# kr4b/pigs

Measured on AMD Instinct MI355X. Metric: sample-points/sec (fwd + 1st + 2nd derivatives, fused), higher is better.
Workload: dtype f32; 1 GPU; c3: 65536 Gaussians x 1024x1024 grid, 1024 rows x 1024 points per GPU, d=2, c=1, kappa=0.5, orders 0-2; gaussians=65536, points_per_gpu=1048576, step=preprocess (cold: nothing reused) + fused forward (orders 0..2)

## Files before the change

pigs_amd/csrc/plan_forward.h:

```cpp
#pragma once
#include "plan_lists.h"

#ifndef PIGS_FWD_WAVES
#define PIGS_FWD_WAVES 8
#endif
#ifndef PIGS_FWD_WG_WAVES
#define PIGS_FWD_WG_WAVES 4
#endif
#ifndef PIGS_FWD_UNROLL
#define PIGS_FWD_UNROLL 2
#endif

namespace pigs {

struct Rec {
    float mu[2], con[3], v[2];
};

template <int STRIDE, typename Body>
__device__ __forceinline__ void walk_point(const PlanView& pv, float x, float y, int i, Body&& body) {
    const GaussGrid gg = pv.params->gg;
    const uint32_t level_mask = pv.params->level_mask;
    for (int l = 0; l < pv.L; ++l) {
        if (!(level_mask >> l & 1u)) continue;
        const int G = pv.G0 >> l;
        const float inv_s = gg.inv_s0 * __builtin_amdgcn_ldexpf(1.f, -l);
        const float gmax = (float)(G - 1);
        const int cx = (int)clampf(floorf((x - gg.ox) * inv_s), 0.f, gmax);
        const int cy = (int)clampf(floorf((y - gg.oy) * inv_s), 0.f, gmax);
        const int cx0 = cx > 0 ? cx - 1 : 0, cx1 = cx < G - 1 ? cx + 1 : G - 1;
        const int cy0 = cy > 0 ? cy - 1 : 0, cy1 = cy < G - 1 ? cy + 1 : G - 1;
        const int csh = level_shift((uint32_t)(G * G));
        uint32_t j0[3], j1[3];
#pragma unroll
        for (int r = 0; r < 3; ++r) {
            const int yy = cy0 + r;
            const uint32_t row = (uint32_t)((yy <= cy1 ? yy : cy1) * G);
            j0[r] = pv.starts[pv.level_off[l] + ((row + (uint32_t)cx0) << csh)];
            j1[r] = yy <= cy1 ? pv.starts[pv.level_off[l] + ((row + (uint32_t)cx1 + 1u) << csh)] : j0[r];
        }
#pragma unroll
        for (int r = 0; r < 3; ++r)
            for (uint32_t j = j0[r] + (uint32_t)i; j < j1[r]; j += STRIDE) body(j, pv.rec[2 * (size_t)j], pv.rec[2 * (size_t)j + 1]);
    }
}
template <typename Body>
__device__ __forceinline__ void walk_point_instep(const PlanView& pv, float x, float y, int i, Body&& body) {
    const GaussGrid gg = pv.params->gg;
    const uint32_t level_mask = pv.params->level_mask;
    for (int l = 0; l < pv.L; ++l) {
        if (!(level_mask >> l & 1u)) continue;
        const int G = pv.G0 >> l;
        const float inv_s = gg.inv_s0 * __builtin_amdgcn_ldexpf(1.f, -l);
        const float gmax = (float)(G - 1);
        const int cx = (int)clampf(floorf((x - gg.ox) * inv_s), 0.f, gmax);
        const int cy = (int)clampf(floorf((y - gg.oy) * inv_s), 0.f, gmax);
        const int cx0 = cx > 0 ? cx - 1 : 0, cx1 = cx < G - 1 ? cx + 1 : G - 1;
        const int cy0 = cy > 0 ? cy - 1 : 0, cy1 = cy < G - 1 ? cy + 1 : G - 1;
        const int csh = level_shift((uint32_t)(G * G));
        uint32_t j0[3], j1[3];
#pragma unroll
        for (int r = 0; r < 3; ++r) {
            const int yy = cy0 + r;
            const uint32_t row = (uint32_t)((yy <= cy1 ? yy : cy1) * G);
            j0[r] = pv.starts[pv.level_off[l] + ((row + (uint32_t)cx0) << csh)];
            j1[r] = yy <= cy1 ? pv.starts[pv.level_off[l] + ((row + (uint32_t)cx1 + 1u) << csh)] : j0[r];
        }
#pragma unroll
        for (int r = 0; r < 3; ++r) {
            uint32_t len = j1[r] - j0[r];
#pragma unroll
            for (int o = 16; o < 64; o <<= 1) len = max(len, (uint32_t)__shfl_xor((int)len, o));
            len = (uint32_t)__builtin_amdgcn_readfirstlane((int)len);
            for (uint32_t o = 0; o < len; o += 16u) {
                const uint32_t j = j0[r] + o + (uint32_t)i;
                const bool have = j < j1[r];
                const size_t jj = have ? j : pv.N;
                body(have, (uint32_t)jj, pv.rec[2 * jj], pv.rec[2 * jj + 1]);
            }
        }
    }
}
__device__ __forceinline__ float pair_q(const float4 A, const float4 B, float x, float y) {
    const float dx = x - A.x, dy = y - A.y;
    return A.z * dx * dx + (2.f * A.w * dx + B.x * dy) * dy;
}
__device__ __forceinline__ Rec make_rec(const float4 A, const float4 B) {
    Rec r;
    r.mu[0] = A.x; r.mu[1] = A.y; r.con[0] = A.z; r.con[1] = A.w; r.con[2] = B.x;
    r.v[0] = B.y; r.v[1] = B.z;
    return r;
}

template <int STEP, bool WIDE, typename Step, typename RangesMask>
__device__ __forceinline__ void for_each_step(const PlanView& pv, uint32_t tile, int lane, Step&& step,
                                              RangesMask&& ranges_mask) {
    const uint32_t hdr = pv.hdr[(size_t)tile * TILE_HDR_WORDS];
    const uint32_t count = hdr & TILE_COUNT_MASK;
    const uint32_t* slab = pv.tlist + (size_t)tile * pv.list_cap;
    if ((hdr >> TILE_MODE_SHIFT) == TILE_MODE_LIST) {
        for (uint32_t e0 = 0; e0 < count; e0 += STEP) {
            const bool have = lane < STEP && e0 + (uint32_t)lane < count;
            const uint32_t e = have ? slab[e0 + lane] : 0u;
            step(e & LIST_IDX_MASK, WIDE ? (e >> LIST_WIDE_SHIFT) & 15u : e >> LIST_NARROW_SHIFT, have);
        }
    } else if ((hdr >> TILE_MODE_SHIFT) == TILE_MODE_GROUPS) {
        for (uint32_t g = 0; g < 4; ++g) {
            const uint32_t ng = pv.hdr[(size_t)tile * TILE_HDR_WORDS + 1 + g];
            const uint32_t* gl = pv.glist + ((size_t)tile * 4 + g) * pv.list_cap;
            for (uint32_t e0 = 0; e0 < ng; e0 += STEP) {
                const bool have = lane < STEP && e0 + (uint32_t)lane < ng;
                step(have ? gl[e0 + lane] : 0u, have ? 1u << g : 0u, have);
            }
        }
    } else {
        auto mask = ranges_mask();
        for (uint32_t r = 0; r < count; ++r) {
            const uint32_t j0 = slab[2 * r], len = slab[2 * r + 1];
            for (uint32_t o = 0; o < len; o += STEP) {
                const bool have = lane < STEP && o + (uint32_t)lane < len;
                const uint32_t idx = have ? j0 + o + (uint32_t)lane : j0;
                step(idx, mask(idx, have), have);
            }
        }
    }
}

#ifndef PIGS_GROUP_CAP
#define PIGS_GROUP_CAP 32
#endif
constexpr int GROUP_CAP = PIGS_GROUP_CAP;
static_assert(GROUP_CAP >= 8 && GROUP_CAP % PIGS_FWD_UNROLL == 0, "queue capacity");

struct FwdLds {
    static constexpr int GSTRIDE = GROUP_CAP * 32 + 32;
    float4 rec[(4 * GSTRIDE + PIGS_FWD_UNROLL * 32) / 16];
};

typedef float f4v __attribute__((ext_vector_type(4)));
typedef float f2v __attribute__((ext_vector_type(2)));

__device__ __forceinline__ uint32_t lds_addr(const void* p) {
    return (uint32_t)(uintptr_t)(const __attribute__((address_space(3))) void*)p;
}
template <int C> struct LdsRec;
template <> struct LdsRec<1> { f4v a; f2v b; };
template <> struct LdsRec<2> { f4v a; f4v b; };
template <int OFF>
__device__ __forceinline__ void lds_rec_issue(LdsRec<1>& r, uint32_t addr) {
    asm volatile("ds_read_b128 %0, %2 offset:%3\n\tds_read_b64 %1, %2 offset:%4"
                 : "=v"(r.a), "=v"(r.b) : "v"(addr), "i"(OFF), "i"(OFF + 16));
}
template <int OFF>
__device__ __forceinline__ void lds_rec_issue(LdsRec<2>& r, uint32_t addr) {
    asm volatile("ds_read_b128 %0, %2 offset:%3\n\tds_read_b128 %1, %2 offset:%4"
                 : "=v"(r.a), "=v"(r.b) : "v"(addr), "i"(OFF), "i"(OFF + 16));
}
template <int C>
__device__ __forceinline__ void lds_rec_wait(LdsRec<C>* r) {
    asm volatile("s_waitcnt lgkmcnt(0)" : "+v"(r[0].a), "+v"(r[0].b), "+v"(r[1].a), "+v"(r[1].b));
}
template <int C>
__device__ __forceinline__ Rec rec_of(const LdsRec<C>& x) {
    Rec r;
    r.mu[0] = x.a.x; r.mu[1] = x.a.y; r.con[0] = x.a.z; r.con[1] = x.a.w; r.con[2] = x.b.x; r.v[0] = x.b.y;
    if constexpr (C == 2) r.v[1] = x.b.z;
    else r.v[1] = 0.f;
    return r;
}

template <int C, int MASK>
__device__ __forceinline__ void evaluate_rows(float* acc, const float* s, const FwdLds& lds, int rows, int lane,
                                              const RzOf<float, MASK>& rz) {
    static_assert(PIGS_FWD_UNROLL == 2, "two rows per register set");
    uint32_t q = lds_addr(lds.rec) + (uint32_t)(lane >> 4) * FwdLds::GSTRIDE;
    LdsRec<C> ra[2], rb[2];
    auto eval2 = [&](const LdsRec<C>* r) {
#pragma unroll
        for (int u = 0; u < 2; ++u) {
            const Rec x = rec_of<C>(r[u]);
            fwd_accumulate<float, 2, C, MASK>(acc, s, x.mu, x.con, x.v, &rz);
        }
    };
    lds_rec_issue<0>(ra[0], q);
    lds_rec_issue<32>(ra[1], q);
    int k = 0;
    for (; k + 4 <= rows; k += 4) {
        lds_rec_wait<C>(ra);
        lds_rec_issue<64>(rb[0], q);
        lds_rec_issue<96>(rb[1], q);
        eval2(ra);
        lds_rec_wait<C>(rb);
        lds_rec_issue<128>(ra[0], q);
        lds_rec_issue<160>(ra[1], q);
        q += 128;
        eval2(rb);
    }
    lds_rec_wait<C>(ra);
    if (k < rows) eval2(ra);
}

template <int C, int MASK>
constexpr int fwd_waves() {
    constexpr int n = FwdLayout<2, C, MASK>::N;
    if (MASK == ORDC) return 7;
    return n > 12 ? 4 : n > 10 ? 5 : (C == 1 && (MASK == 7 || MASK == 19 || MASK == 1 || MASK == ORDR || MASK == ORDG)) ? PIGS_FWD_WAVES : 6;
}
constexpr bool fwd_can_stage(int C, int MASK) { return C == 1 && (MASK == 7 || MASK == 19); }
template <int C, int MASK>
__device__ __forceinline__ void stage_store(const PlanView& pv, const float* acc, uint32_t m) {
    using L = FwdLayout<2, C, MASK>;
    if constexpr (C == 1 && MASK == 7) {
        pv.stage[2 * (size_t)m] = make_float4(acc[L::O0], -acc[L::O1], -acc[L::O1 + 1], acc[L::O2]);
        pv.stage[2 * (size_t)m + 1] = make_float4(acc[L::O2 + 1], acc[L::O2 + 1], acc[L::O2 + 2], 0.f);
    } else if constexpr (C == 1 && MASK == 19) {
        pv.stage[2 * (size_t)m] = make_float4(acc[L::O0], -acc[L::O1], -acc[L::O1 + 1], acc[L::O2]);
    }
}

template <int C, int MASK>
__device__ __forceinline__ void forward_points_quad(const PlanView& pv, const SamplesView& sv, uint32_t tile, uint32_t quad, int lane,
                                                    float q_f, float* __restrict__ o0, float* __restrict__ o1,
                                                    float* __restrict__ o2, float* __restrict__ o3, const RzOf<float, MASK>& rz) {
    using L = FwdLayout<2, C, MASK>;
    const int row = lane >> 4, i = lane & 15;
    const uint32_t m = tile * TILE_POINTS + quad * 4u + (uint32_t)row;
    const bool valid = m < sv.M;
    const SPoint sp = tile_point(sv, point_order(sv), tile, quad * 4u + (uint32_t)row);
    const float s[2] = {sp.x, sp.y};
    float acc[L::N];
#pragma unroll
    for (int k = 0; k < L::N; ++k) acc[k] = 0.f;
    walk_point<16>(pv, sp.x, sp.y, i, [&](uint32_t, const float4 A, const float4 B) {
        if (!(pair_q(A, B, sp.x, sp.y) > q_f)) {
            const Rec r = make_rec(A, B);
            fwd_accumulate<float, 2, C, MASK>(acc, s, r.mu, r.con, r.v, &rz);
        }
    });
#pragma unroll
    for (int k = 0; k < L::N; ++k) {
#pragma unroll
        for (int o = 1; o < 16; o <<= 1) acc[k] += __shfl_xor(acc[k], o);
    }
    if (i == 0 && valid) {
        if (fwd_can_stage(C, MASK) && pv.stage) stage_store<C, MASK>(pv, acc, sp.m);
        else fwd_store<float, 2, C, MASK, false>(acc, (int64_t)sp.m, o0, o1, o2, o3, &rz);
    }
}

template <int C, int MASK>
__device__ __forceinline__ void forward_tile(const PlanView& pv, const SamplesView& sv, uint32_t tile, int lane, FwdLds& lds,
                                             float* __restrict__ o0, float* __restrict__ o1, float* __restrict__ o2,
                                             float* __restrict__ o3, const RzOf<float, MASK>& rz) {
    using L = FwdLayout<2, C, MASK>;
    constexpr int U = PIGS_FWD_UNROLL;
    constexpr bool CAN_STAGE = fwd_can_stage(C, MASK);
    __builtin_amdgcn_s_setprio(3);
    char* const qbase = (char*)lds.rec;
    const uint32_t m = tile * TILE_POINTS + (uint32_t)lane;
    const bool valid = m < sv.M;
    const int g = lane >> 4, i = lane & 15;
    asm volatile("" ::"s"(sv.params), "s"(sv.M), "s"(pv.hdr), "s"(pv.glist), "s"(pv.list_cap));
    const PointOrderWords pw = point_order_words(sv);
    const uint32_t* hd = pv.hdr + (size_t)tile * TILE_HDR_WORDS;
    uint32_t zero = 0u;
    asm("" : "+v"(zero));
    const uint32_t h0v = hd[zero];
    const uint32_t ngv = hd[1 + g];
    const uint32_t* gl = pv.glist + ((size_t)tile * 4 + g) * pv.list_cap;
    uint32_t e0 = gl[(uint32_t)i < pv.list_cap ? i : 0], e1 = gl[16u + (uint32_t)i < pv.list_cap ? 16 + i : 0];
    const SPoint sp = tile_point(sv, point_order(pw), tile, (uint32_t)lane);
    const uint32_t h0 = (uint32_t)__builtin_amdgcn_readfirstlane((int)h0v);
    const float s[2] = {sp.x, sp.y};
    float acc[L::N];
#pragma unroll
    for (int k = 0; k < L::N; ++k) acc[k] = 0.f;
    auto chunk = [&](int rows, auto&& index_of) {
        static_assert(GROUP_CAP == 32, "two rounds of 16 records per chunk");
        rows = __builtin_amdgcn_readfirstlane((rows + U - 1) / U * U);
        const uint32_t j0 = index_of(0, i), j1 = index_of(1, 16 + i);
        const float4 A0 = pv.rec[2 * (size_t)j0], B0 = pv.rec[2 * (size_t)j0 + 1];
        float4 A1 = A0, B1 = B0;
        if (rows > 16) { A1 = pv.rec[2 * (size_t)j1]; B1 = pv.rec[2 * (size_t)j1 + 1]; }
        float4* dst = (float4*)(qbase + g * FwdLds::GSTRIDE + i * 32);
        wave_lds_fence();
        dst[0] = A0;
        *(float2*)(dst + 1) = make_float2(B0.x, B0.y);
        if constexpr (C == 2) *(float2*)((char*)(dst + 1) + 8) = make_float2(B0.z, 0.f);
        if (rows > 16) {
            dst[32] = A1;
            *(float2*)(dst + 33) = make_float2(B1.x, B1.y);
            if constexpr (C == 2) *(float2*)((char*)(dst + 33) + 8) = make_float2(B1.z, 0.f);
        }
        wave_lds_fence();
        __builtin_amdgcn_s_setprio(0);
        evaluate_rows<C, MASK>(acc, s, lds, rows, lane, rz);
        __builtin_amdgcn_s_setprio(3);
    };
    if ((h0 >> TILE_MODE_SHIFT) == TILE_MODE_POINTS) {
        return;
    } else if ((h0 >> TILE_MODE_SHIFT) != TILE_MODE_RANGES) {
        const uint32_t ng = ngv;
        const uint32_t n0 = (uint32_t)__builtin_amdgcn_readlane((int)ngv, 0), n1 = (uint32_t)__builtin_amdgcn_readlane((int)ngv, 16);
        const uint32_t n2 = (uint32_t)__builtin_amdgcn_readlane((int)ngv, 32), n3 = (uint32_t)__builtin_amdgcn_readlane((int)ngv, 48);
        uint32_t nmax = n0 > n1 ? n0 : n1;
        nmax = n2 > nmax ? n2 : nmax;
        nmax = n3 > nmax ? n3 : nmax;
        for (uint32_t base = 0; base < nmax; base += GROUP_CAP) {
            const int rows = (int)(nmax - base < GROUP_CAP ? nmax - base : GROUP_CAP);
            chunk(rows, [&](int round, int p) { return base + p < ng ? (round == 0 ? e0 : e1) : pv.N; });
            if (base + GROUP_CAP < nmax) {
                const uint32_t p0 = base + GROUP_CAP + (uint32_t)i, p1 = p0 + 16u;
                e0 = gl[p0 < pv.list_cap ? p0 : 0u];
                e1 = gl[p1 < pv.list_cap ? p1 : 0u];
            }
        }
    } else {
        const uint32_t* slab = pv.tlist + (size_t)tile * pv.list_cap;
        const uint32_t count = h0 & TILE_COUNT_MASK;
        const float INF = __builtin_huge_valf();
        const float q_f = pv.params->q_f;
        float x0 = valid ? sp.x : INF, x1 = valid ? sp.x : -INF, y0 = valid ? sp.y : INF, y1 = valid ? sp.y : -INF;
        row_box_dpp(x0, x1, y0, y1);
        const bool row_has_points = x0 <= x1;
        float4* const q = (float4*)(qbase + g * FwdLds::GSTRIDE);
        int qn = 0;
        auto drain = [&]() {
            int rows = qn;
#pragma unroll
            for (int o = 16; o < 64; o <<= 1) rows = max(rows, __shfl_xor(rows, o));
            rows = __builtin_amdgcn_readfirstlane((rows + U - 1) / U * U);
            wave_lds_fence();
            for (int k = qn + i; k < rows; k += 16) {
                q[2 * k] = make_float4(0.f, 0.f, 0.f, 0.f);
                q[2 * k + 1] = make_float4(0.f, 0.f, 0.f, 0.f);
            }
            wave_lds_fence();
            if (rows > 0) {
                __builtin_amdgcn_s_setprio(0);
                evaluate_rows<C, MASK>(acc, s, lds, rows, lane, rz);
                __builtin_amdgcn_s_setprio(3);
            }
            qn = 0;
        };
        for (uint32_t r = 0; r < count; ++r) {
            const uint32_t j0 = slab[2 * r], len = slab[2 * r + 1];
            for (uint32_t base = 0; base < len; base += 16) {
                const bool in = base + (uint32_t)i < len;
                const size_t j = in ? j0 + base + (uint32_t)i : pv.N;
                const float4 A = pv.rec[2 * j], B = pv.rec[2 * j + 1];
                const bool hit = in && row_has_points && ellipse_reaches_rect(ellipse_of(A, B.x), x0, y0, x1, y1, q_f);
                const uint32_t rm = (uint32_t)(__ballot(hit) >> (16 * g)) & 0xffffu;
                if (hit) {
                    const int k = qn + __builtin_popcount(rm & ((1u << i) - 1u));
                    q[2 * k] = A;
                    *(float2*)(q + 2 * k + 1) = make_float2(B.x, B.y);
                    if constexpr (C == 2) *(float2*)((char*)(q + 2 * k + 1) + 8) = make_float2(B.z, 0.f);
                }
                qn += __builtin_popcount(rm);
                if (__any(qn > GROUP_CAP - 16)) drain();
            }
        }
        drain();
    }
    const uint32_t m_other = (uint32_t)__shfl_xor((int)sp.m, 1);
    const uint32_t dist = sp.m > m_other ? sp.m - m_other : m_other - sp.m;
    const bool stream = __builtin_popcountll(__ballot(valid && dist == 1u)) >= 48;
    if (CAN_STAGE && pv.stage) {
        if (valid) stage_store<C, MASK>(pv, acc, sp.m);
    } else if (valid) {
        if (stream) {
            fwd_store<float, 2, C, MASK, true>(acc, (int64_t)sp.m, o0, o1, o2, o3, &rz);
            asm volatile("" ::: "memory");
        } else {
            fwd_store<float, 2, C, MASK, false>(acc, (int64_t)sp.m, o0, o1, o2, o3, &rz);
        }
    }
}

template <int C, int MASK>
__global__ __launch_bounds__(64 * PIGS_FWD_WG_WAVES, (fwd_waves<C, MASK>())) void tile_forward_kernel(
    PlanView pv, SamplesView sv, float* __restrict__ o0, float* __restrict__ o1, float* __restrict__ o2,
    float* __restrict__ o3, RzOf<float, MASK> rz) {
    constexpr uint32_t FW = PIGS_FWD_WG_WAVES;
    __shared__ FwdLds lds_all[FW];
    const int lane = threadIdx.x & 63;
    const int wave = __builtin_amdgcn_readfirstlane(threadIdx.x >> 6);
    const uint32_t nmain = (sv.ntiles + FW - 1u) / FW;
    constexpr uint32_t NHELP = POINT_HELPER_BLOCKS * 4u / FW;
    static_assert(NHELP % 8u == 0u, "the main workgroups keep their XCD");
    if (blockIdx.x < NHELP) {
        const uint32_t n = pv.params->n_points;
        if (n == 0u) return;
        const float q_f = pv.params->q_f;
        const uint32_t hw = blockIdx.x * FW + (uint32_t)wave, nhw = NHELP * FW;
        for (uint32_t qd = hw; qd < n * 16u; qd += nhw)
            forward_points_quad<C, MASK>(pv, sv, pv.ptiles[qd >> 4], qd & 15u, lane, q_f, o0, o1, o2, o3, rz);
        return;
    }
    const uint32_t tile = xcd_block_chunk<PIGS_XCD_CHUNK * 4 / FW>(nmain, blockIdx.x - NHELP) * FW + (uint32_t)wave;
    if (tile >= sv.ntiles) return;
    forward_tile<C, MASK>(pv, sv, tile, lane, lds_all[wave], o0, o1, o2, o3, rz);
}

template <int C, int MASK>
__global__ __launch_bounds__(256) void plan_lists_forward_kernel(ListArgs a, float* __restrict__ o0, float* __restrict__ o1,
                                                                 float* __restrict__ o2, float* __restrict__ o3, RzOf<float, MASK> rz) {
    __shared__ ListsLds<LISTS_TPW> lds_all[4];
    static_assert(sizeof(FwdLds) <= sizeof(ListsLds<LISTS_TPW>), "the forward's queues live in the list build's LDS");
    const int lane = threadIdx.x & 63;
    const int wave = __builtin_amdgcn_readfirstlane(threadIdx.x >> 6);
    lists_strip_cover(a);
    const uint32_t tile0 = lists_tile0<LISTS_TPW>(wave);
    const uint32_t ntiles = a.sv.ntiles;
    if (tile0 >= ntiles) return;
    build_block_lists<LISTS_TPW>(a, lds_all[wave], tile0, lane);
    __builtin_amdgcn_fence(__ATOMIC_RELEASE, "workgroup");
    __builtin_amdgcn_fence(__ATOMIC_ACQUIRE, "workgroup");
    FwdLds& flds = *reinterpret_cast<FwdLds*>(&lds_all[wave]);
    for (int t = 0; t < LISTS_TPW; ++t) {
        const uint32_t tile = tile0 + (uint32_t)t;
        if (tile >= ntiles) break;
        const uint32_t h0 = __hip_atomic_load(a.pv.hdr + (size_t)tile * TILE_HDR_WORDS, __ATOMIC_RELAXED, __HIP_MEMORY_SCOPE_WORKGROUP);
        if ((h0 >> TILE_MODE_SHIFT) == TILE_MODE_POINTS) {
            for (uint32_t quad = 0; quad < 16u; ++quad) forward_points_quad<C, MASK>(a.pv, a.sv, tile, quad, lane, a.q_f, o0, o1, o2, o3, rz);
        } else {
            forward_tile<C, MASK>(a.pv, a.sv, tile, lane, flds, o0, o1, o2, o3, rz);
        }
    }
}

template <int MASK>
__global__ __launch_bounds__(256) void stage_to_outputs_kernel(const float4* __restrict__ stage, uint32_t M, float* __restrict__ o0,
                                                               float* __restrict__ o1, float* __restrict__ o2) {
    const uint32_t m = blockIdx.x * 256 + threadIdx.x;
    if (m >= M) return;
    const float4 a = stage[2 * (size_t)m];
    if (o0) __builtin_nontemporal_store(a.x, &o0[m]);
    if (o1) { __builtin_nontemporal_store(a.y, &o1[2 * (size_t)m]); __builtin_nontemporal_store(a.z, &o1[2 * (size_t)m + 1]); }
    if constexpr (MASK == 7) {
        const float4 b = stage[2 * (size_t)m + 1];
        if (o2) {
            float* h = o2 + 4 * (size_t)m;
            __builtin_nontemporal_store(a.w, h); __builtin_nontemporal_store(b.x, h + 1);
            __builtin_nontemporal_store(b.y, h + 2); __builtin_nontemporal_store(b.z, h + 3);
        }
    } else {
        if (o2) __builtin_nontemporal_store(a.w, &o2[m]);
    }
}

}
```

Before: 22.70 billion sample-points/s.

## Stream Gaussian records into LDS via async global_load_lds with double-buffered rounds

Replaces the register-staged global-to-LDS copy of Gaussian records with direct global_load_lds DMA into an interleaved, split A/B layout. Rounds of 16 records are double-buffered, so the next round's load overlaps evaluation of the current one. The LDS layout changes to rows of four groups, and the list-index assignment moves from lane>>4 groups to lane&3 groups. It also adds an occupancy hint of 5 to the lists kernel. The split layout always copies the full 32-byte record including padding, and the vmcnt(0) waits may serialize other loads.

After: 22.86 billion sample-points/s, median of 6. About the same (+0.7%).

```diff
diff --git a/pigs_amd/csrc/plan_forward.h b/pigs_amd/csrc/plan_forward.h
--- a/pigs_amd/csrc/plan_forward.h
+++ b/pigs_amd/csrc/plan_forward.h
@@ -130,11 +130,14 @@
 #define PIGS_GROUP_CAP 32
 #endif
 constexpr int GROUP_CAP = PIGS_GROUP_CAP;
-static_assert(GROUP_CAP >= 8 && GROUP_CAP % PIGS_FWD_UNROLL == 0, "queue capacity");
+static_assert(GROUP_CAP == 32 && PIGS_FWD_UNROLL == 2, "two rounds of 16 records per queue, two rows per register set");
 
 struct FwdLds {
-    static constexpr int GSTRIDE = GROUP_CAP * 32 + 32;
-    float4 rec[(4 * GSTRIDE + PIGS_FWD_UNROLL * 32) / 16];
+    static constexpr int ROUND = 16;
+    static constexpr int ROW = 4 * 16;
+    static constexpr int SLAB = ROUND * ROW;
+    static constexpr int BOFF = GROUP_CAP / ROUND * SLAB;
+    float4 rec[(2 * BOFF + PIGS_FWD_UNROLL * ROW) / 16];
 };
 
 typedef float f4v __attribute__((ext_vector_type(4)));
@@ -149,12 +152,12 @@
 template <int OFF>
 __device__ __forceinline__ void lds_rec_issue(LdsRec<1>& r, uint32_t addr) {
     asm volatile("ds_read_b128 %0, %2 offset:%3\n\tds_read_b64 %1, %2 offset:%4"
-                 : "=v"(r.a), "=v"(r.b) : "v"(addr), "i"(OFF), "i"(OFF + 16));
+                 : "=v"(r.a), "=v"(r.b) : "v"(addr), "i"(OFF), "i"(OFF + FwdLds::BOFF));
 }
 template <int OFF>
 __device__ __forceinline__ void lds_rec_issue(LdsRec<2>& r, uint32_t addr) {
     asm volatile("ds_read_b128 %0, %2 offset:%3\n\tds_read_b128 %1, %2 offset:%4"
-                 : "=v"(r.a), "=v"(r.b) : "v"(addr), "i"(OFF), "i"(OFF + 16));
+                 : "=v"(r.a), "=v"(r.b) : "v"(addr), "i"(OFF), "i"(OFF + FwdLds::BOFF));
 }
 template <int C>
 __device__ __forceinline__ void lds_rec_wait(LdsRec<C>* r) {
@@ -169,11 +172,21 @@
     return r;
 }
 
-template <int C, int MASK>
-__device__ __forceinline__ void evaluate_rows(float* acc, const float* s, const FwdLds& lds, int rows, int lane,
+__device__ __forceinline__ void lds_round_dma(const float4* rec, FwdLds& lds, int round, uint32_t j) {
+    typedef const __attribute__((address_space(1))) void* gptr;
+    typedef __attribute__((address_space(3))) void* lptr;
+    const float4* src = rec + 2 * (size_t)j;
+    char* dst = (char*)lds.rec + round * FwdLds::SLAB;
+    __builtin_amdgcn_global_load_lds((gptr)src, (lptr)dst, 16, 0, 0);
+    __builtin_amdgcn_global_load_lds((gptr)src, (lptr)(dst + FwdLds::BOFF - 16), 16, 16, 0);
+}
+__device__ __forceinline__ void lds_dma_wait() { asm volatile("s_waitcnt vmcnt(0)" ::: "memory"); }
+
+template <int C, int MASK>
+__device__ __forceinline__ void evaluate_rows(float* acc, const float* s, const FwdLds& lds, int row0, int rows, int lane,
                                               const RzOf<float, MASK>& rz) {
-    static_assert(PIGS_FWD_UNROLL == 2, "two rows per register set");
-    uint32_t q = lds_addr(lds.rec) + (uint32_t)(lane >> 4) * FwdLds::GSTRIDE;
+    constexpr int R = FwdLds::ROW;
+    uint32_t q = lds_addr(lds.rec) + (uint32_t)row0 * R + (uint32_t)(lane >> 4) * 16u;
     LdsRec<C> ra[2], rb[2];
     auto eval2 = [&](const LdsRec<C>* r) {
 #pragma unroll
@@ -183,17 +196,17 @@
         }
     };
     lds_rec_issue<0>(ra[0], q);
-    lds_rec_issue<32>(ra[1], q);
+    lds_rec_issue<R>(ra[1], q);
     int k = 0;
     for (; k + 4 <= rows; k += 4) {
         lds_rec_wait<C>(ra);
-        lds_rec_issue<64>(rb[0], q);
-        lds_rec_issue<96>(rb[1], q);
+        lds_rec_issue<2 * R>(rb[0], q);
+        lds_rec_issue<3 * R>(rb[1], q);
         eval2(ra);
         lds_rec_wait<C>(rb);
-        lds_rec_issue<128>(ra[0], q);
-        lds_rec_issue<160>(ra[1], q);
-        q += 128;
+        lds_rec_issue<4 * R>(ra[0], q);
+        lds_rec_issue<5 * R>(ra[1], q);
+        q += 4 * R;
         eval2(rb);
     }
     lds_rec_wait<C>(ra);
@@ -260,60 +273,56 @@
     const uint32_t m = tile * TILE_POINTS + (uint32_t)lane;
     const bool valid = m < sv.M;
     const int g = lane >> 4, i = lane & 15;
+    const int kq = lane >> 2, gq = lane & 3;
     asm volatile("" ::"s"(sv.params), "s"(sv.M), "s"(pv.hdr), "s"(pv.glist), "s"(pv.list_cap));
     const PointOrderWords pw = point_order_words(sv);
     const uint32_t* hd = pv.hdr + (size_t)tile * TILE_HDR_WORDS;
     uint32_t zero = 0u;
     asm("" : "+v"(zero));
     const uint32_t h0v = hd[zero];
-    const uint32_t ngv = hd[1 + g];
-    const uint32_t* gl = pv.glist + ((size_t)tile * 4 + g) * pv.list_cap;
-    uint32_t e0 = gl[(uint32_t)i < pv.list_cap ? i : 0], e1 = gl[16u + (uint32_t)i < pv.list_cap ? 16 + i : 0];
+    const uint32_t ngv = hd[1 + gq];
+    const uint32_t* gl = pv.glist + ((size_t)tile * 4 + gq) * pv.list_cap;
+    uint32_t e0 = gl[(uint32_t)kq < pv.list_cap ? kq : 0], e1 = gl[16u + (uint32_t)kq < pv.list_cap ? 16 + kq : 0];
     const SPoint sp = tile_point(sv, point_order(pw), tile, (uint32_t)lane);
     const uint32_t h0 = (uint32_t)__builtin_amdgcn_readfirstlane((int)h0v);
     const float s[2] = {sp.x, sp.y};
     float acc[L::N];
 #pragma unroll
     for (int k = 0; k < L::N; ++k) acc[k] = 0.f;
-    auto chunk = [&](int rows, auto&& index_of) {
-        static_assert(GROUP_CAP == 32, "two rounds of 16 records per chunk");
-        rows = __builtin_amdgcn_readfirstlane((rows + U - 1) / U * U);
-        const uint32_t j0 = index_of(0, i), j1 = index_of(1, 16 + i);
-        const float4 A0 = pv.rec[2 * (size_t)j0], B0 = pv.rec[2 * (size_t)j0 + 1];
-        float4 A1 = A0, B1 = B0;
-        if (rows > 16) { A1 = pv.rec[2 * (size_t)j1]; B1 = pv.rec[2 * (size_t)j1 + 1]; }
-        float4* dst = (float4*)(qbase + g * FwdLds::GSTRIDE + i * 32);
-        wave_lds_fence();
-        dst[0] = A0;
-        *(float2*)(dst + 1) = make_float2(B0.x, B0.y);
-        if constexpr (C == 2) *(float2*)((char*)(dst + 1) + 8) = make_float2(B0.z, 0.f);
-        if (rows > 16) {
-            dst[32] = A1;
-            *(float2*)(dst + 33) = make_float2(B1.x, B1.y);
-            if constexpr (C == 2) *(float2*)((char*)(dst + 33) + 8) = make_float2(B1.z, 0.f);
-        }
-        wave_lds_fence();
+    auto evaluate = [&](int row0, int rows) {
         __builtin_amdgcn_s_setprio(0);
-        evaluate_rows<C, MASK>(acc, s, lds, rows, lane, rz);
+        evaluate_rows<C, MASK>(acc, s, lds, row0, rows, lane, rz);
         __builtin_amdgcn_s_setprio(3);
     };
     if ((h0 >> TILE_MODE_SHIFT) == TILE_MODE_POINTS) {
         return;
     } else if ((h0 >> TILE_MODE_SHIFT) != TILE_MODE_RANGES) {
         const uint32_t ng = ngv;
-        const uint32_t n0 = (uint32_t)__builtin_amdgcn_readlane((int)ngv, 0), n1 = (uint32_t)__builtin_amdgcn_readlane((int)ngv, 16);
-        const uint32_t n2 = (uint32_t)__builtin_amdgcn_readlane((int)ngv, 32), n3 = (uint32_t)__builtin_amdgcn_readlane((int)ngv, 48);
+        const uint32_t n0 = (uint32_t)__builtin_amdgcn_readlane((int)ngv, 0), n1 = (uint32_t)__builtin_amdgcn_readlane((int)ngv, 1);
+        const uint32_t n2 = (uint32_t)__builtin_amdgcn_readlane((int)ngv, 2), n3 = (uint32_t)__builtin_amdgcn_readlane((int)ngv, 3);
         uint32_t nmax = n0 > n1 ? n0 : n1;
         nmax = n2 > nmax ? n2 : nmax;
         nmax = n3 > nmax ? n3 : nmax;
-        for (uint32_t base = 0; base < nmax; base += GROUP_CAP) {
-            const int rows = (int)(nmax - base < GROUP_CAP ? nmax - base : GROUP_CAP);
-            chunk(rows, [&](int round, int p) { return base + p < ng ? (round == 0 ? e0 : e1) : pv.N; });
-            if (base + GROUP_CAP < nmax) {
-                const uint32_t p0 = base + GROUP_CAP + (uint32_t)i, p1 = p0 + 16u;
-                e0 = gl[p0 < pv.list_cap ? p0 : 0u];
-                e1 = gl[p1 < pv.list_cap ? p1 : 0u];
-            }
+        auto index_of = [&](uint32_t e, uint32_t p) { return p < ng ? e : pv.N; };
+        auto landed = [&]() {
+            lds_dma_wait();
+            asm volatile("" ::"v"(sp.x), "v"(sp.y), "v"(sp.m));
+        };
+        if (nmax > 0u) {
+            wave_lds_fence();
+            lds_round_dma(pv.rec, lds, 0, index_of(e0, (uint32_t)kq));
+            landed();
+        }
+        for (uint32_t base = 0; base < nmax; base += FwdLds::ROUND) {
+            const int rows = __builtin_amdgcn_readfirstlane((int)(nmax - base < FwdLds::ROUND ? (nmax - base + U - 1) / U * U : FwdLds::ROUND));
+            const uint32_t next = base + FwdLds::ROUND;
+            if (next < nmax) {
+                lds_round_dma(pv.rec, lds, (int)(next & FwdLds::ROUND) / FwdLds::ROUND, index_of(e1, next + (uint32_t)kq));
+                const uint32_t p = next + FwdLds::ROUND + (uint32_t)kq;
+                if (next + FwdLds::ROUND < nmax) e1 = gl[p < pv.list_cap ? p : 0u];
+            }
+            evaluate((int)(base & FwdLds::ROUND), rows);
+            landed();
         }
     } else {
         const uint32_t* slab = pv.tlist + (size_t)tile * pv.list_cap;
@@ -323,7 +332,7 @@
         float x0 = valid ? sp.x : INF, x1 = valid ? sp.x : -INF, y0 = valid ? sp.y : INF, y1 = valid ? sp.y : -INF;
         row_box_dpp(x0, x1, y0, y1);
         const bool row_has_points = x0 <= x1;
-        float4* const q = (float4*)(qbase + g * FwdLds::GSTRIDE);
+        char* const q = qbase + g * 16;
         int qn = 0;
         auto drain = [&]() {
             int rows = qn;
@@ -332,15 +341,11 @@
             rows = __builtin_amdgcn_readfirstlane((rows + U - 1) / U * U);
             wave_lds_fence();
             for (int k = qn + i; k < rows; k += 16) {
-                q[2 * k] = make_float4(0.f, 0.f, 0.f, 0.f);
-                q[2 * k + 1] = make_float4(0.f, 0.f, 0.f, 0.f);
+                *(float4*)(q + k * FwdLds::ROW) = make_float4(0.f, 0.f, 0.f, 0.f);
+                *(float4*)(q + k * FwdLds::ROW + FwdLds::BOFF) = make_float4(0.f, 0.f, 0.f, 0.f);
             }
             wave_lds_fence();
-            if (rows > 0) {
-                __builtin_amdgcn_s_setprio(0);
-                evaluate_rows<C, MASK>(acc, s, lds, rows, lane, rz);
-                __builtin_amdgcn_s_setprio(3);
-            }
+            if (rows > 0) evaluate(0, rows);
             qn = 0;
         };
         for (uint32_t r = 0; r < count; ++r) {
@@ -353,9 +358,9 @@
                 const uint32_t rm = (uint32_t)(__ballot(hit) >> (16 * g)) & 0xffffu;
                 if (hit) {
                     const int k = qn + __builtin_popcount(rm & ((1u << i) - 1u));
-                    q[2 * k] = A;
-                    *(float2*)(q + 2 * k + 1) = make_float2(B.x, B.y);
-                    if constexpr (C == 2) *(float2*)((char*)(q + 2 * k + 1) + 8) = make_float2(B.z, 0.f);
+                    *(float4*)(q + k * FwdLds::ROW) = A;
+                    *(float2*)(q + k * FwdLds::ROW + FwdLds::BOFF) = make_float2(B.x, B.y);
+                    if constexpr (C == 2) *(float2*)(q + k * FwdLds::ROW + FwdLds::BOFF + 8) = make_float2(B.z, 0.f);
                 }
                 qn += __builtin_popcount(rm);
                 if (__any(qn > GROUP_CAP - 16)) drain();
@@ -404,7 +409,7 @@
 }
 
 template <int C, int MASK>
-__global__ __launch_bounds__(256) void plan_lists_forward_kernel(ListArgs a, float* __restrict__ o0, float* __restrict__ o1,
+__global__ __launch_bounds__(256, 5) void plan_lists_forward_kernel(ListArgs a, float* __restrict__ o0, float* __restrict__ o1,
                                                                  float* __restrict__ o2, float* __restrict__ o3, RzOf<float, MASK> rz) {
     __shared__ ListsLds<LISTS_TPW> lds_all[4];
     static_assert(sizeof(FwdLds) <= sizeof(ListsLds<LISTS_TPW>), "the forward's queues live in the list build's LDS");
```
